# zjykzj/YOLOv4

Measured on AMD Instinct MI355X. Metric: images/sec fwd+bwd @608x608 bs=64 per GPU (YOLOv4 training step: forward + YOLOLoss + backward), higher is better.
Workload: dtype f32

## Files before the change

yolov4_amd/csrc/conv_f16x2.hip:

```cpp
#include <stdlib.h>
#include "common.h"
#include <cstdlib>
#include "conv_geom.h"

namespace {

using y4::ConvGeom;
using y4::WgradGeom;

typedef _Float16 f16x8 __attribute__((ext_vector_type(8)));
typedef _Float16 f16x2v __attribute__((ext_vector_type(2)));
typedef unsigned int u32x2 __attribute__((ext_vector_type(2)));

__device__ __host__ __forceinline__ unsigned f16x2_scale_exp(unsigned amax_bits) {
    const unsigned e = (amax_bits >> 23) & 0xffu;
    if (e == 0u || e == 255u) return 127u;
    int se = 268 - (int)e;
    if (se < 2) se = 2;
    if (se > 252) se = 252;
    return (unsigned)se;
}
__device__ __forceinline__ float f16x2_scale(const unsigned* amax) {
    return __uint_as_float(f16x2_scale_exp(amax ? *amax : 0u) << 23);
}
// ... 676 lines not shown
#pragma unroll
    for (int i = 0; i < NB; ++i) {
        const int slot = tid + 256 * i;
        const int row = slot >> 3, ch = slot & 3, bpl = (slot >> 2) & 1;
        const bool ok = row < BN && (n0 + row) < g.N;
        b_off[i] = ok ? (unsigned)(n0 + row) * (unsigned)g.K * 4u + (unsigned)(slot & 7) * 16u : OOB;
        b_lds[i] = row < BN ? bpl * BN * ROWB + row * ROWB + ((ch ^ lds_swz<MS>(row)) << 4) : -1;
    }
    const int CC = g.Cs / 32;
    const int S = 9 * CC;
    u32x4 rb[NB];
    int ld_s = 0;
    auto load_b = [&]() {
        const int cc = ld_s / 9, tap = ld_s - cc * 9;
        const unsigned koff = (unsigned)(tap * CC + cc) * 128u;
#pragma unroll
        for (int i = 0; i < NB; ++i) rb[i] = __builtin_amdgcn_raw_buffer_load_b128(wt_rsrc, (int)b_off[i], (int)koff, 0);
        ++ld_s;
    };
    auto store_b = [&](int buf) {
        unsigned char* bs = bsm + buf * BSTAGE;
#pragma unroll
        for (int i = 0; i < NB; ++i)
            if (b_lds[i] >= 0) {
                *reinterpret_cast<u32x4*>(bs + b_lds[i]) = rb[i];
            }
    };
    auto stage_patch = [&](int cc) {
        f32x4 ra[PP];
#pragma unroll
        for (int p = 0; p < PP; ++p) ra[p] = y4_buf_load4(src_rsrc, a_off[p], (unsigned)cc * 128u);
#pragma unroll
        for (int p = 0; p < PP; ++p) {
            if (a_lds[p] < 0) continue;
            f32x4 v = ra[p];
            if (TRANSPOSED && g.Cs_valid != g.Cs) {
#pragma unroll
                for (int e = 0; e < 4; ++e)
                    if (cc * 32 + kc * 4 + e >= g.Cs_valid) v[e] = 0.f;
            }
            u32x2 hi, lo;
            split2x4(v, sa, hi, lo);
            *reinterpret_cast<u32x2*>(smem_b + a_lds[p]) = hi;
            *reinterpret_cast<u32x2*>(smem_b + HALO_ROWS * ROWB + a_lds[p]) = lo;
        }
    };

    accv acc0[TM][TN], acc1[TM][TN];
#pragma unroll
    for (int i = 0; i < TM; ++i)
#pragma unroll
        for (int j = 0; j < TN; ++j)
#pragma unroll
            for (int e = 0; e < ACCN; ++e) { acc0[i][j][e] = 0.f; acc1[i][j][e] = 0.f; }

    const int fr = lane & (MS - 1), fq = lane / MS;
    const int fswb = lds_swz<MS>(fr);
    const int b_row = (wn * WTN + fr) * ROWB;
    int a_rel[TM];
#pragma unroll
    for (int i = 0; i < TM; ++i) {
        int il = wm * WTM + i * MS + fr;
        if (il >= cnt) il = cnt - 1;
        const int pix = i0 + il;
        const int h = pix / W, w = pix - h * W;
        a_rel[i] = h * Wp + w - p_lo;
    }

    auto compute = [&](int buf, int tap) {
        const unsigned char* bs = bsm + buf * BSTAGE;
        const int r = tap / 3, q = tap - r * 3;
        const int toff = TRANSPOSED ? (2 - r) * Wp + (2 - q) : r * Wp + q;
        constexpr int KSN = MS == 32 ? 2 : 1;
#pragma unroll
        for (int ks = 0; ks < KSN; ++ks) {
            const int cb = MS == 32 ? 2 * ks + fq : fq;
            const int cob = (cb ^ fswb) << 4;
            f16x8 fb[TN][2];
#pragma unroll
            for (int j = 0; j < TN; ++j)
#pragma unroll
                for (int pl = 0; pl < 2; ++pl)
                    fb[j][pl] = *reinterpret_cast<const f16x8*>(bs + pl * BN * ROWB + b_row + j * MS * ROWB + cob);
#pragma unroll
            for (int i = 0; i < TM; ++i) {
                const int row = a_rel[i] + toff;
                const int ao = row * ROWB + ((cb ^ lds_swz<MS>(row)) << 4);
                const f16x8 fa0 = *reinterpret_cast<const f16x8*>(smem_b + ao);
                const f16x8 fa1 = *reinterpret_cast<const f16x8*>(smem_b + HALO_ROWS * ROWB + ao);
#pragma unroll
                for (int j = 0; j < TN; ++j) {
                    if constexpr (MS == 32) {
                        acc1[i][j] = __builtin_amdgcn_mfma_f32_32x32x16_f16(fa1, fb[j][0], acc1[i][j], 0, 0, 0);
                        acc1[i][j] = __builtin_amdgcn_mfma_f32_32x32x16_f16(fa0, fb[j][1], acc1[i][j], 0, 0, 0);
                        acc0[i][j] = __builtin_amdgcn_mfma_f32_32x32x16_f16(fa0, fb[j][0], acc0[i][j], 0, 0, 0);
                    } else {
                        acc1[i][j] = __builtin_amdgcn_mfma_f32_16x16x32_f16(fa1, fb[j][0], acc1[i][j], 0, 0, 0);
                        acc1[i][j] = __builtin_amdgcn_mfma_f32_16x16x32_f16(fa0, fb[j][1], acc1[i][j], 0, 0, 0);
                        acc0[i][j] = __builtin_amdgcn_mfma_f32_16x16x32_f16(fa0, fb[j][0], acc0[i][j], 0, 0, 0);
                    }
                }
            }
        }
    };

    load_b();
    store_b(0);
    if (S > 1) load_b();
    for (int s = 0; s < S; ++s) {
        const int cc = s / 9, tap = s - cc * 9;
        if (tap == 0) {
            stage_patch(cc);
            __syncthreads();
        }
        if (s + 1 < S) store_b((s + 1) & 1);
        if (s + 2 < S) load_b();
        compute(s & 1, tap);
        __syncthreads();
    }

    const float un = f16x2_unscale(g.src_amax) * f16x2_unscale(g.wt_amax);
    const float un1 = un * (1.0f / 2048.0f);
    const long long mbase = (long long)b * HW + i0;
    unsigned out_max = 0u;
    bool vec = false;
    if constexpr (MS == 16 && WTN == 64) {
        vec = (g.N & 3) == 0 && (g.ldd & 3) == 0 && (reinterpret_cast<uintptr_t>(g.dst) & 15) == 0 &&
              (!g.res || ((g.ldr & 3) == 0 && (reinterpret_cast<uintptr_t>(g.res) & 15) == 0)) &&
              (!g.scale || (reinterpret_cast<uintptr_t>(g.scale) & 15) == 0) && (!g.shift || (reinterpret_cast<uintptr_t>(g.shift) & 15) == 0);
    }
#pragma unroll
    for (int j = 0; j < TN; ++j)
#pragma unroll
        for (int i = 0; i < TM; ++i)
#pragma unroll
            for (int e = 0; e < ACCN; ++e) {
                const int rl = wm * WTM + i * MS + (MS == 32 ? (e & 3) + 8 * (e >> 2) + 4 * fq : 4 * fq + e);
                acc0[i][j][e] = rl < cnt ? acc0[i][j][e] * un + acc1[i][j][e] * un1 : 0.f;
            }
    if (vec) {
        constexpr int EP = WTN + 4;
        static_assert(4 * WTM * EP * 4 <= 2 * HALO_ROWS * ROWB + 2 * 2 * BN * ROWB, "wave patches must fit the staging buffers");
        float* patch = reinterpret_cast<float*>(smem_b) + wave * (WTM * EP);
#pragma unroll
        for (int j = 0; j < TN; ++j)
#pragma unroll
            for (int i = 0; i < TM; ++i)
#pragma unroll
                for (int e = 0; e < ACCN; ++e) patch[(i * MS + 4 * fq + e) * EP + j * MS + fr] = acc0[i][j][e];
        const int c4 = (lane & 15) * 4;
        const int nv = n0 + wn * WTN + c4;
        const bool nok4 = nv < g.N;
        f32x4 sc4 = {1.f, 1.f, 1.f, 1.f}, sh4 = {0.f, 0.f, 0.f, 0.f};
        if (g.scale && nok4) sc4 = *reinterpret_cast<const f32x4*>(g.scale + nv);
        if (g.shift && nok4) sh4 = *reinterpret_cast<const f32x4*>(g.shift + nv);
#pragma unroll
        for (int it = 0; it < WTM / 4; it += 4) {
            f32x4 rr4[4];
#pragma unroll
            for (int u = 0; u < 4; ++u) {
                const int rl = wm * WTM + (it + u) * 4 + (lane >> 4);
                rr4[u] = (g.res && nok4 && rl < cnt) ? *reinterpret_cast<const f32x4*>(g.res + (mbase + rl) * g.ldr + nv)
                                                    : f32x4{0.f, 0.f, 0.f, 0.f};
            }
#pragma unroll
            for (int u = 0; u < 4; ++u) {
                const int row = (it + u) * 4 + (lane >> 4);
                const int rl = wm * WTM + row;
                f32x4 v = *reinterpret_cast<const f32x4*>(patch + row * EP + c4);
                if (nok4 && rl < cnt) {
#pragma unroll
                    for (int q = 0; q < 4; ++q) {
                        float t = v[q] * sc4[q] + sh4[q];
                        t = y4_act(t, g.act);
                        t += rr4[u][q];
                        v[q] = t;
                        const unsigned vb = __float_as_uint(t) & 0x7fffffffu;
                        if (vb < 0x7f800000u && vb > out_max) out_max = vb;
                    }
                    *reinterpret_cast<f32x4*>(g.dst + (mbase + rl) * g.ldd + nv) = v;
                }
            }
        }
    } else
#pragma unroll
    for (int j = 0; j < TN; ++j) {
        const int n = n0 + wn * WTN + j * MS + fr;
        const bool nok = n < g.N;
        const float sc = (g.scale && nok) ? g.scale[n] : 1.0f;
        const float sh = (g.shift && nok) ? g.shift[n] : 0.0f;
#pragma unroll
        for (int i = 0; i < TM; ++i) {
            float rr[ACCN];
#pragma unroll
            for (int e = 0; e < ACCN; ++e) {
                const int rl = wm * WTM + i * MS + (MS == 32 ? (e & 3) + 8 * (e >> 2) + 4 * fq : 4 * fq + e);
                rr[e] = (g.res && nok && rl < cnt) ? g.res[(mbase + rl) * g.ldr + n] : 0.f;
            }
#pragma unroll
            for (int e = 0; e < ACCN; ++e) {
                const int rl = wm * WTM + i * MS + (MS == 32 ? (e & 3) + 8 * (e >> 2) + 4 * fq : 4 * fq + e);
                const bool rok = rl < cnt;
                const float raw = acc0[i][j][e];
                if (nok && rok) {
                    float v = raw * sc + sh;
                    v = y4_act(v, g.act);
                    v += rr[e];
                    g.dst[(mbase + rl) * g.ldd + n] = v;
                    const unsigned vb = __float_as_uint(v) & 0x7fffffffu;
                    if (vb < 0x7f800000u && vb > out_max) out_max = vb;
                }
            }
        }
    }
    if (!TRANSPOSED && g.dst_amax) {
#pragma unroll
        for (int off = 32; off > 0; off >>= 1) {
            const unsigned o = (unsigned)__shfl_xor((int)out_max, off, 64);
            out_max = o > out_max ? o : out_max;
        }
        if (lane == 0 && out_max > __hip_atomic_load(g.dst_amax, __ATOMIC_RELAXED, __HIP_MEMORY_SCOPE_AGENT)) atomicMax(g.dst_amax, out_max);
    }
    float* const colsums = TRANSPOSED ? nullptr : g.stats;
    if (colsums) {
        __syncthreads();
        float* red = reinterpret_cast<float*>(smem_b);
#pragma unroll
        for (int j = 0; j < TN; ++j) {
            float cs = 0.f, css = 0.f;
#pragma unroll
            for (int i = 0; i < TM; ++i)
#pragma unroll
                for (int e = 0; e < ACCN; ++e) {
                    const float v = acc0[i][j][e];
                    cs += v;
                    css += v * v;
                }
            if constexpr (MS == 16) {
                cs += __shfl_xor(cs, 16, 64);
                css += __shfl_xor(css, 16, 64);
            }
            cs += __shfl_xor(cs, 32, 64);
            css += __shfl_xor(css, 32, 64);
            if (fq == 0) {
                const int c = wn * WTN + j * MS + fr;
                red[(wm * BN + c) * 2 + 0] = cs;
                red[(wm * BN + c) * 2 + 1] = css;
            }
        }
        __syncthreads();
        for (int c = tid; c < BN; c += 256) {
            float cs = 0.f, css = 0.f;
#pragma unroll
            for (int w = 0; w < WM; ++w) { cs += red[(w * BN + c) * 2]; css += red[(w * BN + c) * 2 + 1]; }
            const int n = n0 + c;
            if (n < g.N) {
                colsums[((long long)mt * 2 + 0) * g.N + n] = cs;
                colsums[((long long)mt * 2 + 1) * g.N + n] = css;
            }
        }
    }
}

int halo_patch_rows(int H, int W) {
    const int HW = H * W, Wp = W + 2;
    int worst = 0;
    for (int i0 = 0; i0 < HW; i0 += 128) {
        const int i1 = (i0 + 127 < HW ? i0 + 127 : HW - 1);
        const int h0 = i0 / W, w0 = i0 % W, h1 = i1 / W, w1 = i1 % W;
        const int n = (h1 + 2) * Wp + (w1 + 2) - (h0 * Wp + w0) + 1;
        if (n > worst) worst = n;
    }
    return worst;
}

bool halo_ok(const ConvGeom& g) {
    static const bool off = getenv("Y4_NO_HALO") != nullptr;
    if (off || g.k != 3 || g.stride != 1 || g.pad != 1 || !g.wt_planes) return false;
    if (g.N <= 64 || g.Cs % 32 != 0 || g.Hd != g.Hs || g.Wd != g.Ws) return false;
    if ((unsigned long long)g.Hs * g.Ws * (unsigned long long)g.lds_ * 4ull >= 0xfffffff0ull) return false;
    return halo_patch_rows(g.Hs, g.Ws) <= HALO_ROWS;
}

template <bool TR, int MS>
int launch_halo_f16x2(const ConvGeom& g0, hipStream_t st, int* nparts) {
    constexpr int BN = 128;
    ConvGeom g = g0;
    const int tiles_per_img = (g.Hs * g.Ws + 127) / 128;
    g.mtiles = g.B * tiles_per_img;
    g.ntiles = (g.N + BN - 1) / BN;
    if ((unsigned long long)g.N * g.K * 4ull >= 0xfffffff0ull) return Y4_ERR_SHAPE;
    g.wt_bytes = (unsigned)((unsigned long long)g.N * g.K * 2ull * 2ull);
    if (nparts) *nparts = g.mtiles;
    const size_t smem = 2ull * HALO_ROWS * ROWB + 2ull * 2 * BN * ROWB;
    auto kern = conv3x3_halo_f16x2<BN, TR, MS>;
    static Y4DynLds lds_attr;
    if (!lds_attr.ensure(reinterpret_cast<const void*>(kern), smem)) return Y4_ERR_LAUNCH;
    y4::note_kernel("conv3x3_halo_f16x2<%d, %s, %d>", BN, TR ? "true" : "false", MS);
    hipLaunchKernelGGL(kern, dim3(g.mtiles * g.ntiles), dim3(256), smem, st, g, tiles_per_img);
    Y4_CHECK_LAUNCH();
    return Y4_OK;
}

template <int KS, int NT, int NW = 4, bool RESB = false, bool PLAIN = false>
__global__ __launch_bounds__(NW * 64, NW == 4 ? 2 : 1) void conv1x1_stream_f16x2(const ConvGeom g) {
    constexpr int NTHR = NW * 64, TROWS = NW * 32;
    constexpr int K = KS * 16;
    constexpr int PITCH = K * 2 + 16;
    constexpr int N32 = NT * 32;
    extern __shared__ __attribute__((aligned(16))) unsigned char smem_b[];
    const int tid = threadIdx.x, lane = tid & 63, wave = tid >> 6;
    const int fr = lane & 31, fh = lane >> 5;
    {
        constexpr int CPR = K / 8;
        const unsigned char* wp = reinterpret_cast<const unsigned char*>(g.wt_planes);
        for (int i = tid; i < 2 * N32 * CPR; i += NTHR) {
            const int pl = i / (N32 * CPR);
            const int rem = i - pl * (N32 * CPR);
            const int row = rem / CPR, ch = rem - row * CPR;
            u32x4 v = {0u, 0u, 0u, 0u};
            if (row < g.N) v = *reinterpret_cast<const u32x4*>(wp + (size_t)row * (K * 4) + (ch >> 2) * 128 + pl * 64 + (ch & 3) * 16);
            *reinterpret_cast<u32x4*>(smem_b + (pl * N32 + row) * PITCH + ch * 16) = v;
        }
    }
    __syncthreads();

    const __amdgpu_buffer_rsrc_t src_rsrc = y4_make_rsrc(g.src, (unsigned)g.src_total_bytes);
    const unsigned pix_bytes = (unsigned)g.lds_ * 4u;
    const int mtiles = g.mtiles;
    const float sa = f16x2_scale(g.src_amax);
    const float un = f16x2_unscale(g.src_amax) * f16x2_unscale(g.wt_amax);
    const float un1 = un * (1.0f / 2048.0f);
    constexpr int KH = KS == 8 ? 4 : KS;
    f32x4 ra0[KH][2], ra1[KH][2];
    auto load = [&](f32x4 (&ra)[KH][2], int tile, int ks0) {
        const int m = tile * TROWS + wave * 32 + fr;
        const unsigned off = m < g.M ? (unsigned)m * pix_bytes + (unsigned)fh * 32u : 0xffffffffu;
#pragma unroll
        for (int ks = 0; ks < KH; ++ks) {
            ra[ks][0] = y4_buf_load4(src_rsrc, off, (unsigned)(ks0 + ks) * 64u);
            ra[ks][1] = y4_buf_load4(src_rsrc, off, (unsigned)(ks0 + ks) * 64u + 16u);
        }
    };
    float cs[PLAIN ? 1 : NT], css[PLAIN ? 1 : NT];
    float sc[PLAIN ? 1 : NT], sh[PLAIN ? 1 : NT];
    if constexpr (!PLAIN) {
#pragma unroll
        for (int j = 0; j < NT; ++j) {
            cs[j] = 0.f; css[j] = 0.f;
            const int n = j * 32 + fr;
            sc[j] = (g.scale && n < g.N) ? g.scale[n] : 1.0f;
            sh[j] = (g.shift && n < g.N) ? g.shift[n] : 0.0f;
        }
    }
    const unsigned char* b_frag = smem_b + fr * PITCH + fh * 16;
    f32x16 acc0[NT], acc1[NT];
    auto zero_acc = [&]() {
#pragma unroll
        for (int j = 0; j < NT; ++j)
#pragma unroll
            for (int e = 0; e < 16; ++e) { acc0[j][e] = 0.f; acc1[j][e] = 0.f; }
    };
    auto mma = [&](f32x4 (&ra)[KH][2], int ks0) {
        if constexpr (KS == 8) asm volatile("" ::: "memory");
#pragma unroll
        for (int ks = 0; ks < KH; ++ks) {
            f16x8 fah, fal;
            {
                u32x2 h0, l0, h1, l1;
                split2x4(ra[ks][0], sa, h0, l0);
                split2x4(ra[ks][1], sa, h1, l1);
                const u32x4 qh = {h0[0], h0[1], h1[0], h1[1]}, ql = {l0[0], l0[1], l1[0], l1[1]};
                fah = __builtin_bit_cast(f16x8, qh);
                fal = __builtin_bit_cast(f16x8, ql);
            }
#pragma unroll
            for (int j = 0; j < NT; ++j) {
                const f16x8 fbh = *reinterpret_cast<const f16x8*>(b_frag + (j * 32) * PITCH + (ks0 + ks) * 32);
                const f16x8 fbl = *reinterpret_cast<const f16x8*>(b_frag + (N32 + j * 32) * PITCH + (ks0 + ks) * 32);
                acc1[j] = __builtin_amdgcn_mfma_f32_32x32x16_f16(fal, fbh, acc1[j], 0, 0, 0);
                acc1[j] = __builtin_amdgcn_mfma_f32_32x32x16_f16(fah, fbl, acc1[j], 0, 0, 0);
                acc0[j] = __builtin_amdgcn_mfma_f32_32x32x16_f16(fah, fbh, acc0[j], 0, 0, 0);
            }
        }
    };
    unsigned out_max = 0u;
    const unsigned drow_bytes = (unsigned)g.ldd * 4u, rrow_bytes = (unsigned)g.ldr * 4u;
    auto epilogue = [&](int tile) {
        if constexpr (RESB) {
            const long long row0 = (long long)tile * TROWS;
            const unsigned long long rows_left = (unsigned long long)(g.M - row0);
            const unsigned long long dby = rows_left * drow_bytes, rby = rows_left * rrow_bytes;
            const __amdgpu_buffer_rsrc_t drs = y4_make_rsrc(reinterpret_cast<char*>(g.dst) + row0 * (long long)drow_bytes,
                                                            (unsigned)(dby < 0xfffffff0ull ? dby : 0xfffffff0ull));
            const bool has_res = RESB || g.res != nullptr;
            const __amdgpu_buffer_rsrc_t rrs = y4_make_rsrc(has_res ? reinterpret_cast<const char*>(g.res) + row0 * (long long)rrow_bytes : nullptr,
                                                            has_res ? (unsigned)(rby < 0xfffffff0ull ? rby : 0xfffffff0ull) : 0u);
            const int lrow = wave * 32 + 4 * fh;
            const bool rows_in = row0 + TROWS <= g.M;
    #pragma unroll
            for (int j = 0; j < NT; ++j) {
                const int n = j * 32 + fr;
                const bool nok = n < g.N;
                unsigned dvo4[4], rvo4[4];
    #pragma unroll
                for (int q = 0; q < 4; ++q) {
                    dvo4[q] = nok ? (unsigned)(lrow + 8 * q) * drow_bytes + (unsigned)n * 4u : 0xffffffffu;
                    rvo4[q] = nok ? (unsigned)(lrow + 8 * q) * rrow_bytes + (unsigned)n * 4u : 0xffffffffu;
                }
                constexpr int RB = RESB ? 16 : 4;
    #pragma unroll
                for (int eb = 0; eb < 16; eb += RB) {
                    float rr[RB];
                    if (has_res) {
    #pragma unroll
                        for (int ee = 0; ee < RB; ++ee) {
                            const int e = eb + ee;
                            rr[ee] = __builtin_bit_cast(float, __builtin_amdgcn_raw_buffer_load_b32(rrs, (int)(rvo4[e >> 2]), (int)((e & 3) * rrow_bytes), 0));
                        }
                    }
    #pragma unroll
                    for (int ee = 0; ee < RB; ++ee) {
                        const int e = eb + ee;
                        const float raw = acc0[j][e] * un + acc1[j][e] * un1;
                        if constexpr (!PLAIN) { cs[j] += raw; css[j] += raw * raw; }
                        float v = raw;
                        if constexpr (!PLAIN) {
                            v = raw * sc[j] + sh[j];
                            v = y4_act(v, g.act);
                        }
                        if (has_res) v += rr[ee];
                        __builtin_amdgcn_raw_buffer_store_b32(__builtin_bit_cast(unsigned, v), drs, (int)(dvo4[e >> 2]), (int)((e & 3) * drow_bytes), 0);
                        if (g.dst_amax) {
                            const bool ok = nok && (rows_in || row0 + lrow + (e & 3) + 8 * (e >> 2) < g.M);
                            const unsigned vb = __float_as_uint(v) & 0x7fffffffu;
                            if (ok && vb < 0x7f800000u && vb > out_max) out_max = vb;
                        }
                    }
                }
            }
        } else {
            const int mbase = tile * TROWS + wave * 32 + 4 * fh;
    #pragma unroll
            for (int j = 0; j < NT; ++j) {
                const int n = j * 32 + fr;
                const bool nok = n < g.N;
                constexpr int RB = RESB ? (NT <= 2 ? 16 : 8) : 16;
    #pragma unroll
                for (int eb = 0; eb < 16; eb += RB) {
                    float rr[RESB ? RB : 1];
                    if constexpr (RESB) {
    #pragma unroll
                        for (int e = 0; e < RB; ++e) {
                            const int m = mbase + ((eb + e) & 3) + 8 * ((eb + e) >> 2);
                            rr[e] = (g.res && nok && m < g.M) ? g.res[(long long)m * g.ldr + n] : 0.f;
                        }
                    }
    #pragma unroll
                    for (int ee = 0; ee < RB; ++ee) {
                        const int e = eb + ee;
                        const float raw = acc0[j][e] * un + acc1[j][e] * un1;
                        if constexpr (!PLAIN) { cs[j] += raw; css[j] += raw * raw; }
                        const int m = mbase + (e & 3) + 8 * (e >> 2);
                        if (nok && m < g.M) {
                            float v = raw;
                            if constexpr (!PLAIN) {
                                v = raw * sc[j] + sh[j];
                                v = y4_act(v, g.act);
                            }
                            if constexpr (RESB) v += rr[ee];
                            else if (g.res) v += g.res[(long long)m * g.ldr + n];
                            g.dst[(long long)m * g.ldd + n] = v;
                            const unsigned vb = __float_as_uint(v) & 0x7fffffffu;
                            if (vb < 0x7f800000u && vb > out_max) out_max = vb;
                        }
                    }
                }
            }
        }
    };
    int tile = blockIdx.x;
    if (tile < mtiles) load(ra0, tile, 0);
    if constexpr (KS == 8) {
        while (tile < mtiles) {
            load(ra1, tile, KH);
            zero_acc();
            mma(ra0, 0);
            const int tn = tile + gridDim.x;
            if (tn < mtiles) load(ra0, tn, 0);
            mma(ra1, KH);
            epilogue(tile);
            tile = tn;
        }
    } else {
        while (tile < mtiles) {
            const int t1 = tile + gridDim.x;
            if (t1 < mtiles) load(ra1, t1, 0);
            zero_acc(); mma(ra0, 0); epilogue(tile);
            if (t1 >= mtiles) break;
            const int t2 = t1 + gridDim.x;
            if (t2 < mtiles) load(ra0, t2, 0);
            zero_acc(); mma(ra1, 0); epilogue(t1);
            tile = t2;
        }
    }
    if (g.dst_amax) {
#pragma unroll
        for (int off = 32; off > 0; off >>= 1) {
            const unsigned o = (unsigned)__shfl_xor((int)out_max, off, 64);
            out_max = o > out_max ? o : out_max;
        }
        if (lane == 0 && out_max > __hip_atomic_load(g.dst_amax, __ATOMIC_RELAXED, __HIP_MEMORY_SCOPE_AGENT)) atomicMax(g.dst_amax, out_max);
    }
    if (!PLAIN && g.stats) {
        __syncthreads();
        float* red = reinterpret_cast<float*>(smem_b);
#pragma unroll
        for (int j = 0; j < NT; ++j) {
            float a = cs[j], b = css[j];
            a += __shfl_xor(a, 32, 64);
            b += __shfl_xor(b, 32, 64);
            if (fh == 0) { red[(wave * N32 + j * 32 + fr) * 2] = a; red[(wave * N32 + j * 32 + fr) * 2 + 1] = b; }
        }
        __syncthreads();
        for (int c = tid; c < N32; c += NTHR) {
            float a = 0.f, b = 0.f;
#pragma unroll
            for (int w = 0; w < NW; ++w) { a += red[(w * N32 + c) * 2]; b += red[(w * N32 + c) * 2 + 1]; }
            if (c < g.N) {
                g.stats[((long long)blockIdx.x * 2 + 0) * g.N + c] = a;
                g.stats[((long long)blockIdx.x * 2 + 1) * g.N + c] = b;
            }
        }
    }
}

template <int KS, int NT, int NW, bool RESB, bool PLAIN = false>
int launch_stream1x1_f16x2_impl(const ConvGeom& g0, hipStream_t st, int* nparts);
template <int KS, int NT, int NW = 4>
int launch_stream1x1_f16x2(const ConvGeom& g0, hipStream_t st, int* nparts) {
    if constexpr (KS == 8 && NT == 4) {
        if (g0.res && !g0.scale && !g0.shift && !g0.stats && g0.act == Y4_ACT_LINEAR)
            return launch_stream1x1_f16x2_impl<KS, NT, NW, true, true>(g0, st, nparts);
    } else if constexpr (NT <= 2) {
        if (g0.res) return launch_stream1x1_f16x2_impl<KS, NT, NW, true>(g0, st, nparts);
    }
    return launch_stream1x1_f16x2_impl<KS, NT, NW, false>(g0, st, nparts);
}
template <int KS, int NT, int NW, bool RESB, bool PLAIN>
int launch_stream1x1_f16x2_impl(const ConvGeom& g0, hipStream_t st, int* nparts) {
    ConvGeom g = g0;
    g.mtiles = (g.M + NW * 32 - 1) / (NW * 32);
    g.ntiles = 1;
    g.src_total_bytes = (unsigned long long)g.M * (unsigned long long)g.lds_ * 4ull;
    size_t smem = (size_t)2 * NT * 32 * (KS * 32 + 16);
    const size_t red = (size_t)NW * NT * 32 * 2 * sizeof(float);
    if (smem < red) smem = red;
    auto kern = conv1x1_stream_f16x2<KS, NT, NW, RESB, PLAIN>;
    static Y4DynLds lds_attr;
    if (!lds_attr.ensure(reinterpret_cast<const void*>(kern), smem)) return Y4_ERR_LAUNCH;
    const int resident = NW == 8 ? 256 : 512;
    const int grid = g.mtiles < resident ? g.mtiles : resident;
    if (nparts) *nparts = grid;
    y4::note_kernel("conv1x1_stream_f16x2<%d, %d, %d, %s, %s>", KS, NT, NW, RESB ? "true" : "false", PLAIN ? "true" : "false");
    hipLaunchKernelGGL(kern, dim3(grid), dim3(NW * 64), smem, st, g);
    Y4_CHECK_LAUNCH();
    return Y4_OK;
}

bool stream1x1_f16x2_ok(const ConvGeom& g) {
    if (g.k != 1 || g.stride != 1 || !g.wt_planes) return false;
    if (g.Cs != 32 && g.Cs != 64 && g.Cs != 128) return false;
    if (g.Cs_valid != g.Cs || g.N > 128) return false;
    if ((unsigned long long)g.M * (unsigned long long)g.lds_ * 4ull >= 0xfffffff0ull) return false;
    return g.M >= 128 * 1024;
}

int dispatch_stream1x1_f16x2(const ConvGeom& g, hipStream_t st, int* nparts) {
    const int nt = (g.N + 31) / 32;
    switch (g.Cs / 16 * 10 + nt) {
        case 21: return launch_stream1x1_f16x2<2, 1>(g, st, nparts);
        case 22: return launch_stream1x1_f16x2<2, 2>(g, st, nparts);
        case 23: case 24: return launch_stream1x1_f16x2<2, 4>(g, st, nparts);
        case 41: return launch_stream1x1_f16x2<4, 1>(g, st, nparts);
        case 42: return launch_stream1x1_f16x2<4, 2>(g, st, nparts);
        case 43: case 44: return launch_stream1x1_f16x2<4, 4>(g, st, nparts);
        case 81: return launch_stream1x1_f16x2<8, 1>(g, st, nparts);
        case 82: return launch_stream1x1_f16x2<8, 2>(g, st, nparts);
        case 83: case 84: return launch_stream1x1_f16x2<8, 4, 8>(g, st, nparts);
        default: return Y4_ERR_SHAPE;
    }
}

__device__ __forceinline__ void amax_block_commit(unsigned m, unsigned* out) {
    __shared__ unsigned wmax[4];
#pragma unroll
    for (int off = 32; off > 0; off >>= 1) {
        const unsigned o = (unsigned)__shfl_xor((int)m, off, 64);
        m = o > m ? o : m;
    }
    if ((threadIdx.x & 63) == 0) wmax[threadIdx.x >> 6] = m;
    __syncthreads();
    if (threadIdx.x == 0) {
        const unsigned a = wmax[0] > wmax[1] ? wmax[0] : wmax[1], b = wmax[2] > wmax[3] ? wmax[2] : wmax[3];
        const unsigned v = a > b ? a : b;
        if (v > __hip_atomic_load(out, __ATOMIC_RELAXED, __HIP_MEMORY_SCOPE_AGENT)) atomicMax(out, v);
    }
}
__global__ __launch_bounds__(256) void amax_kernel(const float* __restrict__ x, long long ld, long long M, int C,
                                                   unsigned* __restrict__ out) {
    unsigned m = 0u;
    const int C4 = (C + 3) >> 2;
    const long long total = M * C4;
    for (long long i = blockIdx.x * (long long)blockDim.x + threadIdx.x; i < total; i += (long long)gridDim.x * blockDim.x) {
        const long long row = i / C4;
        const int c = (int)(i - row * C4) * 4;
        const f32x4 v = *reinterpret_cast<const f32x4*>(x + row * ld + c);
#pragma unroll
        for (int e = 0; e < 4; ++e) {
            const unsigned b = __float_as_uint(v[e]) & 0x7fffffffu;
            if (c + e < C && b < 0x7f800000u && b > m) m = b;
        }
    }
    amax_block_commit(m, out);
}
__global__ __launch_bounds__(256) void amax_strided_kernel(const float* __restrict__ x, long long ld, long long M, int C,
                                                           unsigned* __restrict__ out) {
    unsigned m = 0u;
    const long long total = M * C;
    for (long long i = blockIdx.x * (long long)blockDim.x + threadIdx.x; i < total; i += (long long)gridDim.x * blockDim.x) {
        const long long row = i / C;
        const unsigned b = __float_as_uint(x[row * ld + (i - row * C)]) & 0x7fffffffu;
        if (b < 0x7f800000u && b > m) m = b;
    }
    amax_block_commit(m, out);
}
__global__ void amax_merge_kernel(unsigned* __restrict__ dst, const unsigned* __restrict__ src) {
    if (threadIdx.x == 0 && blockIdx.x == 0) { const unsigned v = *src; if (v) atomicMax(dst, v); }
}

constexpr int AMAX_PART_MAX = 1024;
__global__ __launch_bounds__(256) void amax_partials_kernel(const float* __restrict__ x, long long n, unsigned* __restrict__ part) {
    __shared__ unsigned wmax[4];
    unsigned m = 0u;
    const long long n4 = n >> 2;
    for (long long i = blockIdx.x * (long long)blockDim.x + threadIdx.x; i < n4; i += (long long)gridDim.x * blockDim.x) {
        const f32x4 v = *reinterpret_cast<const f32x4*>(x + 4 * i);
#pragma unroll
        for (int e = 0; e < 4; ++e) {
            const unsigned b = __float_as_uint(v[e]) & 0x7fffffffu;
            if (b < 0x7f800000u && b > m) m = b;
        }
    }
    if (blockIdx.x == 0 && threadIdx.x < (int)(n & 3)) {
        const unsigned b = __float_as_uint(x[(n4 << 2) + threadIdx.x]) & 0x7fffffffu;
        if (b < 0x7f800000u && b > m) m = b;
    }
#pragma unroll
    for (int off = 32; off > 0; off >>= 1) {
        const unsigned o = (unsigned)__shfl_xor((int)m, off, 64);
        m = o > m ? o : m;
    }
    if ((threadIdx.x & 63) == 0) wmax[threadIdx.x >> 6] = m;
    __syncthreads();
    if (threadIdx.x == 0) {
        const unsigned a = wmax[0] > wmax[1] ? wmax[0] : wmax[1], b = wmax[2] > wmax[3] ? wmax[2] : wmax[3];
        part[blockIdx.x] = a > b ? a : b;
    }
}
__device__ __forceinline__ unsigned amax_fold_partials(const unsigned* __restrict__ part, int nparts, unsigned* __restrict__ out) {
    __shared__ unsigned wmax[4];
    unsigned m = 0u;
    for (int i = threadIdx.x; i < nparts; i += 256) { const unsigned v = part[i]; m = v > m ? v : m; }
#pragma unroll
    for (int off = 32; off > 0; off >>= 1) {
        const unsigned o = (unsigned)__shfl_xor((int)m, off, 64);
        m = o > m ? o : m;
    }
    if ((threadIdx.x & 63) == 0) wmax[threadIdx.x >> 6] = m;
    __syncthreads();
    const unsigned a = wmax[0] > wmax[1] ? wmax[0] : wmax[1], b = wmax[2] > wmax[3] ? wmax[2] : wmax[3];
    const unsigned v = a > b ? a : b;
    if (blockIdx.x == 0 && threadIdx.x == 0) *out = v;
    return v;
}
__global__ __launch_bounds__(256) void f16x2_split_filter_folded_kernel(const float* __restrict__ w, unsigned short* __restrict__ planes,
                                                                        long long n, const unsigned* __restrict__ part, int nparts,
                                                                        unsigned* __restrict__ amax_out) {
    const unsigned amax = amax_fold_partials(part, nparts, amax_out);
    const float s = __uint_as_float(f16x2_scale_exp(amax) << 23);
    for (long long i = blockIdx.x * (long long)blockDim.x + threadIdx.x; i < n; i += (long long)gridDim.x * blockDim.x) {
        unsigned short hi, lo;
        split2(w[i], s, hi, lo);
        const long long o = (i >> 5) * 64 + (i & 31);
        planes[o] = hi;
        planes[o + 32] = lo;
    }
}
__global__ __launch_bounds__(256) void f16x2_split_filter_dual_kernel(const float* __restrict__ w, unsigned short* __restrict__ planes,
                                                                      unsigned short* __restrict__ planes_t, int Cout, int Cin, int kk,
                                                                      int Cout_pad, const unsigned* __restrict__ part, int nparts,
                                                                      unsigned* __restrict__ amax_out, unsigned* __restrict__ amax_out_t,
                                                                      int mirror) {
    const unsigned amax = amax_fold_partials(part, nparts, amax_out);
    if (blockIdx.x == 0 && threadIdx.x == 0) *amax_out_t = amax;
    const float s = __uint_as_float(f16x2_scale_exp(amax) << 23);
    const long long n = (long long)Cout * kk * Cin;
    for (long long i = blockIdx.x * (long long)blockDim.x + threadIdx.x; i < n; i += (long long)gridDim.x * blockDim.x) {
        unsigned short hi, lo;
        split2(w[i], s, hi, lo);
        const long long o = (i >> 5) * 64 + (i & 31);
        planes[o] = hi;
        planes[o + 32] = lo;
    }
    const long long total = (long long)Cin * kk * Cout_pad;
    for (long long i = blockIdx.x * (long long)blockDim.x + threadIdx.x; i < total; i += (long long)gridDim.x * blockDim.x) {
        const int nn = (int)(i % Cout_pad);
        const long long t = i / Cout_pad;
        const int tp = (int)(t % kk);
        const int tap = mirror ? kk - 1 - tp : tp;
        const int c = (int)(t / kk);
        const float v = nn < Cout ? w[((long long)nn * kk + tap) * Cin + c] : 0.0f;
        unsigned short hi, lo;
        split2(v, s, hi, lo);
        const long long o = (i >> 5) * 64 + (i & 31);
        planes_t[o] = hi;
        planes_t[o + 32] = lo;
    }
}
__global__ __launch_bounds__(256) void f16x2_transpose_split_filter_folded_kernel(const float* __restrict__ w,
                                                                                  unsigned short* __restrict__ planes, int Cout, int Cin,
                                                                                  int kk, int Cout_pad, const unsigned* __restrict__ part,
                                                                                  int nparts, unsigned* __restrict__ amax_out, int mirror) {
    const unsigned amax = amax_fold_partials(part, nparts, amax_out);
    const float s = __uint_as_float(f16x2_scale_exp(amax) << 23);
    const long long total = (long long)Cin * kk * Cout_pad;
    for (long long i = blockIdx.x * (long long)blockDim.x + threadIdx.x; i < total;
         i += (long long)gridDim.x * blockDim.x) {
        const int n = (int)(i % Cout_pad);
        const long long t = i / Cout_pad;
        const int tp = (int)(t % kk);
        const int tap = mirror ? kk - 1 - tp : tp;
        const int c = (int)(t / kk);
        const float v = n < Cout ? w[((long long)n * kk + tap) * Cin + c] : 0.0f;
        unsigned short hi, lo;
        split2(v, s, hi, lo);
        const long long o = (i >> 5) * 64 + (i & 31);
        planes[o] = hi;
        planes[o + 32] = lo;
    }
}

constexpr int FP_PARTS = 256;
__global__ __launch_bounds__(256) void f16x2_refresh_filter_kernel(const float* __restrict__ w, unsigned short* __restrict__ planes,
                                                                   long long n, unsigned* part_max, unsigned long long* part_sum,
                                                                   unsigned* hdr) {
    __shared__ unsigned wmax[4];
    __shared__ unsigned long long wsum[4];
    __shared__ int is_last;
    unsigned m = 0u;
    unsigned long long cs = 0ull;
    auto take = [&](const float x, const unsigned long long i) {
        const unsigned bits = __float_as_uint(x);
        cs += (unsigned long long)bits * (2ull * i + 1ull) + 0x9e3779b97f4a7c15ull;
        const unsigned b = bits & 0x7fffffffu;
        if (b < 0x7f800000u && b > m) m = b;
    };
    {
        const long long n4 = n >> 2, stride = (long long)gridDim.x * blockDim.x;
        long long i = blockIdx.x * (long long)blockDim.x + threadIdx.x;
        for (; i + 3 * stride < n4; i += 4 * stride) {
            f32x4 v[4];
#pragma unroll
            for (int u = 0; u < 4; ++u) v[u] = *reinterpret_cast<const f32x4*>(w + 4 * (i + u * stride));
#pragma unroll
            for (int u = 0; u < 4; ++u)
#pragma unroll
                for (int e = 0; e < 4; ++e) take(v[u][e], (unsigned long long)(4 * (i + u * stride) + e));
        }
        for (; i < n4; i += stride) {
            const f32x4 v = *reinterpret_cast<const f32x4*>(w + 4 * i);
#pragma unroll
            for (int e = 0; e < 4; ++e) take(v[e], (unsigned long long)(4 * i + e));
        }
        if (blockIdx.x == 0 && threadIdx.x < (int)(n & 3)) take(w[(n4 << 2) + threadIdx.x], (unsigned long long)((n4 << 2) + threadIdx.x));
    }
#pragma unroll
    for (int off = 32; off > 0; off >>= 1) {
        const unsigned o = (unsigned)__shfl_xor((int)m, off, 64);
        m = o > m ? o : m;
        cs += __shfl_xor(cs, off, 64);
    }
    if ((threadIdx.x & 63) == 0) { wmax[threadIdx.x >> 6] = m; wsum[threadIdx.x >> 6] = cs; }
    __syncthreads();
    if (threadIdx.x == 0) {
        const unsigned a = wmax[0] > wmax[1] ? wmax[0] : wmax[1], b = wmax[2] > wmax[3] ? wmax[2] : wmax[3];
        __hip_atomic_store(part_max + blockIdx.x, a > b ? a : b, __ATOMIC_RELAXED, __HIP_MEMORY_SCOPE_AGENT);
        __hip_atomic_store(part_sum + blockIdx.x, wsum[0] + wsum[1] + wsum[2] + wsum[3], __ATOMIC_RELAXED, __HIP_MEMORY_SCOPE_AGENT);
        asm volatile("s_waitcnt vmcnt(0)" ::: "memory");
        const unsigned t = __hip_atomic_fetch_add(hdr + 5, 1u, __ATOMIC_RELAXED, __HIP_MEMORY_SCOPE_AGENT);
        is_last = t == gridDim.x - 1;
    }
    __syncthreads();
    if (!is_last) return;
    m = 0u; cs = 0ull;
    for (int i = threadIdx.x; i < (int)gridDim.x; i += 256) {
        const unsigned v = __hip_atomic_load(part_max + i, __ATOMIC_RELAXED, __HIP_MEMORY_SCOPE_AGENT);
        m = v > m ? v : m;
        cs += __hip_atomic_load(part_sum + i, __ATOMIC_RELAXED, __HIP_MEMORY_SCOPE_AGENT);
    }
#pragma unroll
    for (int off = 32; off > 0; off >>= 1) {
        const unsigned o = (unsigned)__shfl_xor((int)m, off, 64);
        m = o > m ? o : m;
        cs += __shfl_xor(cs, off, 64);
    }
    __syncthreads();
    if ((threadIdx.x & 63) == 0) { wmax[threadIdx.x >> 6] = m; wsum[threadIdx.x >> 6] = cs; }
    __syncthreads();
    const unsigned a = wmax[0] > wmax[1] ? wmax[0] : wmax[1], b = wmax[2] > wmax[3] ? wmax[2] : wmax[3];
    const unsigned amax = a > b ? a : b;
    const unsigned long long sum = wsum[0] + wsum[1] + wsum[2] + wsum[3];
    const unsigned long long stored = (unsigned long long)hdr[2] | ((unsigned long long)hdr[3] << 32);
    const bool same = hdr[4] == 1u && stored == sum && hdr[0] == amax;
    if (!same) {
        const float s = __uint_as_float(f16x2_scale_exp(amax) << 23);
        for (long long i = threadIdx.x; i < n; i += 256) {
            unsigned short hi, lo;
            split2(w[i], s, hi, lo);
            const long long o = (i >> 5) * 64 + (i & 31);
            planes[o] = hi;
            planes[o + 32] = lo;
        }
    }
    __syncthreads();
    if (threadIdx.x == 0) {
        if (!same) { hdr[0] = amax; hdr[2] = (unsigned)sum; hdr[3] = (unsigned)(sum >> 32); hdr[4] = 1u; }
        hdr[5] = 0u;
    }
}

int g_f16x2_shape = 16;

template <int BM, int BN, int WM, int WN, bool TR, int MS>
int launch_gather_f16x2(const ConvGeom& g0, hipStream_t st) {
    ConvGeom g = g0;
    if (TR && g.stride == 2) {
        int t = 0;
        for (int c = 0; c < 4; ++c) {
            const int ph = (3 - c) >> 1, pw = (3 - c) & 1;
            g.cls_h[ph] = (g.Hd + 1 - ph) / 2;
            g.cls_w[pw] = (g.Wd + 1 - pw) / 2;
            g.cls_tile0[c] = t;
            const long long n = (long long)g.B * g.cls_h[ph] * g.cls_w[pw];
            t += (int)((n + BM - 1) / BM);
        }
        g.cls_tile0[4] = t;
        g.mtiles = t;
    } else {
        g.cls_slot0[0] = 0;
        g.mtiles = (g.M + BM - 1) / BM;
    }
    g.ntiles = (g.N + BN - 1) / BN;
    {
        const unsigned long long img = (unsigned long long)g.Hs * g.Ws * (unsigned long long)g.lds_ * 4ull;
        const unsigned long long wb = (unsigned long long)g.N * g.K * 4ull;
        const unsigned long long imgs_per_tile = (unsigned long long)BM / (unsigned long long)((g.Hd * g.Wd + 3) / 4 > 0 ? (g.Hd * g.Wd + 3) / 4 : 1) + 2;
// ... 182 lines not shown
```

Before: 453.1.

## Transpose 1x1 stream conv epilogue through LDS for row-wise 128-bit stores

Replaces the per-element scattered b32 stores in the 1x1 streaming conv epilogue with a per-wave LDS patch transpose. Each thread then writes 4 contiguous channels with b128 buffer stores and loads the residual as b128 too. Scale and shift are staged in static LDS. The previous PLAIN/RESB specializations are removed in favour of a single ROWS path chosen when N, the leading dimensions and the pointers are 16-byte aligned. This is meant to cut store transactions and improve coalescing, at the cost of extra LDS traffic and static shared memory that may lower occupancy.

```diff
diff --git a/yolov4_amd/csrc/conv_f16x2.hip b/yolov4_amd/csrc/conv_f16x2.hip
--- a/yolov4_amd/csrc/conv_f16x2.hip
+++ b/yolov4_amd/csrc/conv_f16x2.hip
@@ -1002,7 +1002,7 @@
     return Y4_OK;
 }
 
-template <int KS, int NT, int NW = 4, bool RESB = false, bool PLAIN = false>
+template <int KS, int NT, int NW = 4, bool ROWS = true>
 __global__ __launch_bounds__(NW * 64, NW == 4 ? 2 : 1) void conv1x1_stream_f16x2(const ConvGeom g) {
     constexpr int NTHR = NW * 64, TROWS = NW * 32;
     constexpr int K = KS * 16;
@@ -1011,6 +1011,18 @@
     extern __shared__ __attribute__((aligned(16))) unsigned char smem_b[];
     const int tid = threadIdx.x, lane = tid & 63, wave = tid >> 6;
     const int fr = lane & 31, fh = lane >> 5;
+    constexpr int PATCH = 32 * 32;
+    float* patch = nullptr;
+    const float* scsh = nullptr;
+    if constexpr (ROWS) {
+        __shared__ __attribute__((aligned(16))) float ep_lds[NW * PATCH + 2 * N32];
+        patch = ep_lds + wave * PATCH;
+        scsh = ep_lds + NW * PATCH;
+        for (int i = tid; i < N32; i += NTHR) {
+            ep_lds[NW * PATCH + i] = (g.scale && i < g.N) ? g.scale[i] : 1.0f;
+            ep_lds[NW * PATCH + N32 + i] = (g.shift && i < g.N) ? g.shift[i] : 0.0f;
+        }
+    }
     {
         constexpr int CPR = K / 8;
         const unsigned char* wp = reinterpret_cast<const unsigned char*>(g.wt_planes);
@@ -1034,20 +1046,22 @@
     constexpr int KH = KS == 8 ? 4 : KS;
     f32x4 ra0[KH][2], ra1[KH][2];
     auto load = [&](f32x4 (&ra)[KH][2], int tile, int ks0) {
-        const int m = tile * TROWS + wave * 32 + fr;
-        const unsigned off = m < g.M ? (unsigned)m * pix_bytes + (unsigned)fh * 32u : 0xffffffffu;
+        int t = tid;
+        if constexpr (ROWS) asm volatile("" : "+v"(t));
+        const int m = tile * TROWS + (t >> 6) * 32 + (t & 31);
+        const unsigned off = m < g.M ? (unsigned)m * pix_bytes + (unsigned)((t >> 5) & 1) * 32u : 0xffffffffu;
 #pragma unroll
         for (int ks = 0; ks < KH; ++ks) {
             ra[ks][0] = y4_buf_load4(src_rsrc, off, (unsigned)(ks0 + ks) * 64u);
             ra[ks][1] = y4_buf_load4(src_rsrc, off, (unsigned)(ks0 + ks) * 64u + 16u);
         }
     };
-    float cs[PLAIN ? 1 : NT], css[PLAIN ? 1 : NT];
-    float sc[PLAIN ? 1 : NT], sh[PLAIN ? 1 : NT];
-    if constexpr (!PLAIN) {
-#pragma unroll
-        for (int j = 0; j < NT; ++j) {
-            cs[j] = 0.f; css[j] = 0.f;
+    float cs[NT], css[NT];
+    float sc[ROWS ? 1 : NT], sh[ROWS ? 1 : NT];
+#pragma unroll
+    for (int j = 0; j < NT; ++j) {
+        cs[j] = 0.f; css[j] = 0.f;
+        if constexpr (!ROWS) {
             const int n = j * 32 + fr;
             sc[j] = (g.scale && n < g.N) ? g.scale[n] : 1.0f;
             sh[j] = (g.shift && n < g.N) ? g.shift[n] : 0.0f;
@@ -1086,54 +1100,72 @@
     };
     unsigned out_max = 0u;
     const unsigned drow_bytes = (unsigned)g.ldd * 4u, rrow_bytes = (unsigned)g.ldr * 4u;
+    auto sq_rn = [](float x) {
+#pragma clang fp contract(off)
+        return x * x;
+    };
+    auto act4 = [&](f32x4 v) {
+        switch (g.act) {
+            case Y4_ACT_LEAKY: for (int q = 0; q < 4; ++q) v[q] = y4_act_t<Y4_ACT_LEAKY>(v[q]); break;
+            case Y4_ACT_MISH: for (int q = 0; q < 4; ++q) v[q] = y4_act_t<Y4_ACT_MISH>(v[q]); break;
+            case Y4_ACT_RELU: for (int q = 0; q < 4; ++q) v[q] = y4_act_t<Y4_ACT_RELU>(v[q]); break;
+            default: break;
+        }
+        return v;
+    };
     auto epilogue = [&](int tile) {
-        if constexpr (RESB) {
+        if constexpr (ROWS) {
             const long long row0 = (long long)tile * TROWS;
             const unsigned long long rows_left = (unsigned long long)(g.M - row0);
             const unsigned long long dby = rows_left * drow_bytes, rby = rows_left * rrow_bytes;
             const __amdgpu_buffer_rsrc_t drs = y4_make_rsrc(reinterpret_cast<char*>(g.dst) + row0 * (long long)drow_bytes,
                                                             (unsigned)(dby < 0xfffffff0ull ? dby : 0xfffffff0ull));
-            const bool has_res = RESB || g.res != nullptr;
+            const bool has_res = g.res != nullptr;
             const __amdgpu_buffer_rsrc_t rrs = y4_make_rsrc(has_res ? reinterpret_cast<const char*>(g.res) + row0 * (long long)rrow_bytes : nullptr,
                                                             has_res ? (unsigned)(rby < 0xfffffff0ull ? rby : 0xfffffff0ull) : 0u);
-            const int lrow = wave * 32 + 4 * fh;
             const bool rows_in = row0 + TROWS <= g.M;
+            int t = tid;
+            asm volatile("" : "+v"(t));
+            const int prow = (t >> 3) & 7, c4 = (t & 7) * 4;
+            const int lrow = (t >> 6) * 32 + prow;
+            float* pw = patch + (4 * ((t >> 5) & 1)) * 32 + (t & 31);
+            const float* pr = patch + prow * 32 + c4;
+            const unsigned dvo = (unsigned)lrow * drow_bytes + (unsigned)c4 * 4u, rvo = (unsigned)lrow * rrow_bytes + (unsigned)c4 * 4u;
     #pragma unroll
             for (int j = 0; j < NT; ++j) {
-                const int n = j * 32 + fr;
-                const bool nok = n < g.N;
-                unsigned dvo4[4], rvo4[4];
     #pragma unroll
-                for (int q = 0; q < 4; ++q) {
-                    dvo4[q] = nok ? (unsigned)(lrow + 8 * q) * drow_bytes + (unsigned)n * 4u : 0xffffffffu;
-                    rvo4[q] = nok ? (unsigned)(lrow + 8 * q) * rrow_bytes + (unsigned)n * 4u : 0xffffffffu;
+                for (int e = 0; e < 16; ++e) {
+                    const float raw = acc0[j][e] * un + acc1[j][e] * un1;
+                    cs[j] += raw; css[j] += sq_rn(raw);
+                    pw[((e & 3) + 8 * (e >> 2)) * 32] = raw;
                 }
-                constexpr int RB = RESB ? 16 : 4;
+                asm volatile("" : "+v"(cs[j]), "+v"(css[j]));
+                const int nv = j * 32 + c4;
+                const bool nok4 = nv < g.N;
+                const f32x4 sc4 = *reinterpret_cast<const f32x4*>(scsh + nv), sh4 = *reinterpret_cast<const f32x4*>(scsh + N32 + nv);
+                f32x4 rr4[4];
+                if (has_res) {
     #pragma unroll
-                for (int eb = 0; eb < 16; eb += RB) {
-                    float rr[RB];
+                    for (int u = 0; u < 4; ++u)
+                        rr4[u] = y4_buf_load4(rrs, nok4 ? rvo + (unsigned)(8 * u) * rrow_bytes + (unsigned)j * 128u : 0xffffffffu, 0u);
+                }
+    #pragma unroll
+                for (int u = 0; u < 4; ++u) {
+                    f32x4 v = *reinterpret_cast<const f32x4*>(pr + (8 * u) * 32);
+    #pragma unroll
+                    for (int q = 0; q < 4; ++q) v[q] = __builtin_fmaf(v[q], sc4[q], sh4[q]);
+                    v = act4(v);
                     if (has_res) {
     #pragma unroll
-                        for (int ee = 0; ee < RB; ++ee) {
-                            const int e = eb + ee;
-                            rr[ee] = __builtin_bit_cast(float, __builtin_amdgcn_raw_buffer_load_b32(rrs, (int)(rvo4[e >> 2]), (int)((e & 3) * rrow_bytes), 0));
-                        }
+                        for (int q = 0; q < 4; ++q) v[q] += rr4[u][q];
                     }
+                    __builtin_amdgcn_raw_buffer_store_b128(__builtin_bit_cast(u32x4, v), drs,
+                                                           (int)(nok4 ? dvo + (unsigned)(8 * u) * drow_bytes + (unsigned)j * 128u : 0xffffffffu), 0, 0);
+                    if (g.dst_amax) {
+                        const bool ok = nok4 && (rows_in || row0 + lrow + 8 * u < g.M);
     #pragma unroll
-                    for (int ee = 0; ee < RB; ++ee) {
-                        const int e = eb + ee;
-                        const float raw = acc0[j][e] * un + acc1[j][e] * un1;
-                        if constexpr (!PLAIN) { cs[j] += raw; css[j] += raw * raw; }
-                        float v = raw;
-                        if constexpr (!PLAIN) {
-                            v = raw * sc[j] + sh[j];
-                            v = y4_act(v, g.act);
-                        }
-                        if (has_res) v += rr[ee];
-                        __builtin_amdgcn_raw_buffer_store_b32(__builtin_bit_cast(unsigned, v), drs, (int)(dvo4[e >> 2]), (int)((e & 3) * drow_bytes), 0);
-                        if (g.dst_amax) {
-                            const bool ok = nok && (rows_in || row0 + lrow + (e & 3) + 8 * (e >> 2) < g.M);
-                            const unsigned vb = __float_as_uint(v) & 0x7fffffffu;
+                        for (int q = 0; q < 4; ++q) {
+                            const unsigned vb = __float_as_uint(v[q]) & 0x7fffffffu;
                             if (ok && vb < 0x7f800000u && vb > out_max) out_max = vb;
                         }
                     }
@@ -1145,35 +1177,18 @@
             for (int j = 0; j < NT; ++j) {
                 const int n = j * 32 + fr;
                 const bool nok = n < g.N;
-                constexpr int RB = RESB ? (NT <= 2 ? 16 : 8) : 16;
     #pragma unroll
-                for (int eb = 0; eb < 16; eb += RB) {
-                    float rr[RESB ? RB : 1];
-                    if constexpr (RESB) {
-    #pragma unroll
-                        for (int e = 0; e < RB; ++e) {
-                            const int m = mbase + ((eb + e) & 3) + 8 * ((eb + e) >> 2);
-                            rr[e] = (g.res && nok && m < g.M) ? g.res[(long long)m * g.ldr + n] : 0.f;
-                        }
-                    }
-    #pragma unroll
-                    for (int ee = 0; ee < RB; ++ee) {
-                        const int e = eb + ee;
-                        const float raw = acc0[j][e] * un + acc1[j][e] * un1;
-                        if constexpr (!PLAIN) { cs[j] += raw; css[j] += raw * raw; }
-                        const int m = mbase + (e & 3) + 8 * (e >> 2);
-                        if (nok && m < g.M) {
-                            float v = raw;
-                            if constexpr (!PLAIN) {
-                                v = raw * sc[j] + sh[j];
-                                v = y4_act(v, g.act);
-                            }
-                            if constexpr (RESB) v += rr[ee];
-                            else if (g.res) v += g.res[(long long)m * g.ldr + n];
-                            g.dst[(long long)m * g.ldd + n] = v;
-                            const unsigned vb = __float_as_uint(v) & 0x7fffffffu;
-                            if (vb < 0x7f800000u && vb > out_max) out_max = vb;
-                        }
+                for (int e = 0; e < 16; ++e) {
+                    const float raw = acc0[j][e] * un + acc1[j][e] * un1;
+                    cs[j] += raw; css[j] += raw * raw;
+                    const int m = mbase + (e & 3) + 8 * (e >> 2);
+                    if (nok && m < g.M) {
+                        float v = raw * sc[j] + sh[j];
+                        v = y4_act(v, g.act);
+                        if (g.res) v += g.res[(long long)m * g.ldr + n];
+                        g.dst[(long long)m * g.ldd + n] = v;
+                        const unsigned vb = __float_as_uint(v) & 0x7fffffffu;
+                        if (vb < 0x7f800000u && vb > out_max) out_max = vb;
                     }
                 }
             }
@@ -1212,15 +1227,18 @@
         }
         if (lane == 0 && out_max > __hip_atomic_load(g.dst_amax, __ATOMIC_RELAXED, __HIP_MEMORY_SCOPE_AGENT)) atomicMax(g.dst_amax, out_max);
     }
-    if (!PLAIN && g.stats) {
+    if (g.stats) {
         __syncthreads();
         float* red = reinterpret_cast<float*>(smem_b);
+        int t = tid;
+        if constexpr (ROWS) asm volatile("" : "+v"(t));
+        const int rcol = (t >> 6) * N32 + (t & 31);
 #pragma unroll
         for (int j = 0; j < NT; ++j) {
             float a = cs[j], b = css[j];
             a += __shfl_xor(a, 32, 64);
             b += __shfl_xor(b, 32, 64);
-            if (fh == 0) { red[(wave * N32 + j * 32 + fr) * 2] = a; red[(wave * N32 + j * 32 + fr) * 2 + 1] = b; }
+            if ((t & 32) == 0) { red[(rcol + j * 32) * 2] = a; red[(rcol + j * 32) * 2 + 1] = b; }
         }
         __syncthreads();
         for (int c = tid; c < N32; c += NTHR) {
@@ -1235,19 +1253,15 @@
     }
 }
 
-template <int KS, int NT, int NW, bool RESB, bool PLAIN = false>
+template <int KS, int NT, int NW, bool ROWS>
 int launch_stream1x1_f16x2_impl(const ConvGeom& g0, hipStream_t st, int* nparts);
 template <int KS, int NT, int NW = 4>
 int launch_stream1x1_f16x2(const ConvGeom& g0, hipStream_t st, int* nparts) {
-    if constexpr (KS == 8 && NT == 4) {
-        if (g0.res && !g0.scale && !g0.shift && !g0.stats && g0.act == Y4_ACT_LINEAR)
-            return launch_stream1x1_f16x2_impl<KS, NT, NW, true, true>(g0, st, nparts);
-    } else if constexpr (NT <= 2) {
-        if (g0.res) return launch_stream1x1_f16x2_impl<KS, NT, NW, true>(g0, st, nparts);
-    }
-    return launch_stream1x1_f16x2_impl<KS, NT, NW, false>(g0, st, nparts);
-}
-template <int KS, int NT, int NW, bool RESB, bool PLAIN>
+    const bool rows = (g0.N & 3) == 0 && (g0.ldd & 3) == 0 && (reinterpret_cast<uintptr_t>(g0.dst) & 15) == 0 &&
+                      (!g0.res || ((g0.ldr & 3) == 0 && (reinterpret_cast<uintptr_t>(g0.res) & 15) == 0));
+    return rows ? launch_stream1x1_f16x2_impl<KS, NT, NW, true>(g0, st, nparts) : launch_stream1x1_f16x2_impl<KS, NT, NW, false>(g0, st, nparts);
+}
+template <int KS, int NT, int NW, bool ROWS>
 int launch_stream1x1_f16x2_impl(const ConvGeom& g0, hipStream_t st, int* nparts) {
     ConvGeom g = g0;
     g.mtiles = (g.M + NW * 32 - 1) / (NW * 32);
@@ -1256,13 +1270,13 @@
     size_t smem = (size_t)2 * NT * 32 * (KS * 32 + 16);
     const size_t red = (size_t)NW * NT * 32 * 2 * sizeof(float);
     if (smem < red) smem = red;
-    auto kern = conv1x1_stream_f16x2<KS, NT, NW, RESB, PLAIN>;
+    auto kern = conv1x1_stream_f16x2<KS, NT, NW, ROWS>;
     static Y4DynLds lds_attr;
     if (!lds_attr.ensure(reinterpret_cast<const void*>(kern), smem)) return Y4_ERR_LAUNCH;
     const int resident = NW == 8 ? 256 : 512;
     const int grid = g.mtiles < resident ? g.mtiles : resident;
     if (nparts) *nparts = grid;
-    y4::note_kernel("conv1x1_stream_f16x2<%d, %d, %d, %s, %s>", KS, NT, NW, RESB ? "true" : "false", PLAIN ? "true" : "false");
+    y4::note_kernel("conv1x1_stream_f16x2<%d, %d, %d, %s>", KS, NT, NW, ROWS ? "true" : "false");
     hipLaunchKernelGGL(kern, dim3(grid), dim3(NW * 64), smem, st, g);
     Y4_CHECK_LAUNCH();
     return Y4_OK;
```

Result: no change. 457.1, median of 6 (+0.9%).
